# jkxing/EPSM_Mitsuba3

Hardware: AMD Instinct MI355X
Metric: manifold_paths_per_s (higher is better)
Workload: dtype f32

## Files before the change

### epsm_mitsuba3_amd/csrc/epsm_backward_cp.hip

```cpp
#include <stdlib.h>
#include <string.h>

#define EPSM_FAST_RCP64
#include "epsm_fused.h"
#include "epsm_cp_core.h"
#include "epsm_wave_scatter.h"

using namespace epsm;

namespace {

#ifndef EPSM_CP_THREADS
#define EPSM_CP_THREADS 256
#endif
#ifndef EPSM_CP_OCC
#define EPSM_CP_OCC 3
#endif
#ifndef EPSM_CP_ROWS_FLOAT
#define EPSM_CP_ROWS_FLOAT 2064
#endif
#ifndef EPSM_CP_ROWS_FIXED
#define EPSM_CP_ROWS_FIXED 1184
#endif
#ifndef EPSM_CP_QUEUE
#define EPSM_CP_QUEUE 192
#endif
#ifndef EPSM_CP_BLOCKS
#define EPSM_CP_BLOCKS (1 << 20)
#endif
constexpr int kThreads = EPSM_CP_THREADS, kWaves = kThreads / 64, kQueueCap = EPSM_CP_QUEUE;
constexpr int kKeys = 6;
constexpr int kStashFirstItem = 64;
static_assert(kQueueCap - kStashFirstItem >= 128, "the stash needs 128 queue items");

__device__ __forceinline__ int div_small(int lane, int c) {
    const int inv = c == 1 ? 65536 : c == 2 ? 32768 : c == 3 ? 21846 : c == 4 ? 16384 : 13108;
    return (lane * inv) >> 16;
}

__device__ __forceinline__ int up1_bits(int v) { return __builtin_amdgcn_update_dpp(v, v, 0x138, 0xf, 0xf, false); }
__device__ __forceinline__ int down1_bits(int v) { return __builtin_amdgcn_update_dpp(v, v, 0x130, 0xf, 0xf, false); }
__device__ __forceinline__ float up1(float v) { return __int_as_float(up1_bits(__float_as_int(v))); }
__device__ __forceinline__ float down1(float v) { return __int_as_float(down1_bits(__float_as_int(v))); }
__device__ __forceinline__ int up1(int v) { return up1_bits(v); }
__device__ __forceinline__ int down1(int v) { return down1_bits(v); }
__device__ __forceinline__ uint32_t up1(uint32_t v) { return (uint32_t) up1_bits((int) v); }
__device__ __forceinline__ uint32_t down1(uint32_t v) { return (uint32_t) down1_bits((int) v); }
__device__ __forceinline__ V2<float> up1(V2<float> v) { return mk2<float>(up1(v.x), up1(v.y)); }
__device__ __forceinline__ M2<float> up1(M2<float> m) { M2<float> o; o.a = up1(m.a); o.b = up1(m.b); o.c = up1(m.c); o.d = up1(m.d); return o; }
__device__ __forceinline__ V3<float> down1(V3<float> v) { return mk3<float>(down1(v.x), down1(v.y), down1(v.z)); }
__device__ __forceinline__ V3<float> up1(V3<float> v) { return mk3<float>(up1(v.x), up1(v.y), up1(v.z)); }

template <bool PACKED> struct Records {
    const FusedArgs &F;
    const PtrTable &P;
    int64_t i;
    __device__ __forceinline__ cp::Own<float> own(int k) const {
        cp::Own<float> o;
        const VertexPtrs<float> &v = P.v[k - 1];
        const Geo<float> g = load_geo(v, i);
        const Nrm<float> nr = load_nrm(v, i, g.b0, g.b1);
        o.x = g.x; o.e1 = g.e1; o.e2 = g.e2; o.b0 = g.b0; o.b1 = g.b1;
        o.n = nr.n; o.dn1 = nr.dn1; o.dn2 = nr.dn2; o.eta = lds_(v.eta, i); o.light = load3(v.light, i);
        return o;
    }
    __device__ __forceinline__ Geo<float> geo(int k) const { return load_geo(P.v[k - 1], i); }
    __device__ __forceinline__ V3<float> cam() const { return load3(F.g.cam, i); }
    __device__ __forceinline__ uint32_t tri_id(int k) const { return lds_(P.s[k - 1].tri, i); }
    __device__ __forceinline__ void b0b1(int k, float &b0, float &b1) const { b0 = lds_(P.v[k - 1].b0, i); b1 = lds_(P.v[k - 1].b1, i); }
    __device__ __forceinline__ bool emit(int k, uint32_t &etri, float &eb0, float &eb1, float &ew) const {
        const uint32_t *p = P.s[k - 1].emit;
        if (!p) return false;
        const U4 e4 = load_u4(p, i);
        etri = e4.x; eb0 = bits_to_float(e4.y); eb1 = bits_to_float(e4.z); ew = bits_to_float(e4.w);
        return true;
    }
    __device__ __forceinline__ void aux(int k, uint32_t &bid, V3<float> &dhf) const {
        bid = kNoIndex; dhf = zero3<float>();
        if (!F.galpha || !P.s[k - 1].aux) return;
        const U4 a4 = load_u4(P.s[k - 1].aux, i);
        bid = a4.x; dhf = mk3<float>(bits_to_float(a4.y), bits_to_float(a4.z), bits_to_float(a4.w));
    }
    __device__ __forceinline__ uint32_t flag_word() const {
        if (PACKED) return lds_(F.pk_flags, i);
        uint32_t w = 0;
        for (int k = 1; k <= F.K; ++k) {
            const VertexPtrs<float> &v = P.v[k - 1];
            const uint32_t b = lds_(v.bsdf, i);
            w |= (((b & kBsdfDiffuse) ? 1u : 0u) | ((b & kBsdfNull) ? 2u : 0u) | (lds_(v.active, i) ? 4u : 0u) |
                  (lds_(v.active_em, i) ? 8u : 0u) | (lds_(v.ismesh, i) ? 16u : 0u)) << (5 * (k - 1));
        }
        return w;
    }
};

template <typename Table> struct Emitter {
    const FusedArgs &F;
    const Table &T;
    WaveQueue<kQueueCap> &Q;

    template <int ROWS>
    __device__ __forceinline__ void push(bool valid, const uint32_t key[ROWS], const V3<float> val[ROWS]) const {
        Q.template push_rows<ROWS>(T, valid, key, val);
    }
    __device__ __forceinline__ V3<float> fin(V3<float> g) const {
        return mk3<float>(finalize(g.x, F.g.clip), finalize(g.y, F.g.clip), finalize(g.z, F.g.clip));
    }
    __device__ __forceinline__ static bool tri_ok(const U4 &t, int64_t V) {
        return t.x < (uint64_t) V && t.y < (uint64_t) V && t.z < (uint64_t) V;
    }
    __device__ __forceinline__ void rows3(bool v, V3<float> vals[3], uint32_t a, uint32_t b, uint32_t c) const {
        const uint32_t keys[3] = {a, b, c};
        push<3>(v, keys, vals);
    }
    __device__ __forceinline__ void group(bool v, V3<float> g, float w0, float w1, uint32_t a, uint32_t b, uint32_t c) const {
        if (__ballot(v) == 0ull) return;
        V3<float> vals[3] = {g * w0, g * w1, g * (1.f - w0 - w1)};
        rows3(v, vals, a, b, c);
    }
    __device__ __forceinline__ void vertex(bool on, bool live, bool d1, V3<float> Gx, V3<float> gn, V3<float> gm, V3<float> glight,
                                           V3<float> gdiff, V3<float> dp, V3<float> n, V3<float> e1, V3<float> e2, float b0, float b1,
                                           float nb0, float nb1, uint32_t bid, V3<float> dhf, float eb0, float eb1, float ew,
                                           const U4 &t, const U4 &tn, const U4 &er, const U4 &sh, const U4 &ts) const {
        const V3<float> z = zero3<float>();
        const bool idx_ok = tri_ok(t, F.V), pos_ok = idx_ok && (t.w & kModePos);
        gn = fin(gn);
        const bool gn_on = on && idx_ok && nz3(gn);
        const float sgn = (t.w & kModeFlip) ? -1.f : 1.f;
        const V3<float> dpf = d1 ? fin(dp) : z;
        {
            const float b2 = 1.f - b0 - b1;
            V3<float> P[3] = {on ? fin(Gx * b0) : z, on ? fin(Gx * b1) : z, on ? fin(Gx * b2) : z};
            if (gn_on && !(t.w & kModeVertexNormals) && pos_ok) {
                const V3<float> d0 = e2 - e1, d1_ = -e1;
                const V3<float> cr = cross(d0, d1_);
                const float il = rsqrt_(dot(cr, cr));
                const V3<float> ch = cr * il;
                const V3<float> cb = (gn - ch * dot(ch, gn)) * (il * sgn);
                const V3<float> d0b = cross(d1_, cb), d1b = cross(cb, d0);
                P[1] = P[1] + d0b; P[2] = P[2] + d1b; P[0] = P[0] - (d0b + d1b);
            }
            if (d1) { P[0] = P[0] + dpf * b0; P[1] = P[1] + dpf * b1; P[2] = P[2] + dpf * b2; }
            const bool v = pos_ok && (nz3(P[0]) || nz3(P[1]) || nz3(P[2]));
            if (__ballot(v) != 0ull) rows3(v, P, t.x, t.y, t.z);
        }
        {
            V3<float> pg = z;
            if (gn_on && (t.w & kModeVertexNormals) && (t.w & kModeNrm)) {
                const float il = rsqrt_(dot(n, n));
                const V3<float> sh_ = n * il;
                pg = (gn - sh_ * dot(sh_, gn)) * (il * sgn);
            }
            const uint32_t V32 = (uint32_t) F.V;
            group(nz3(pg), pg, b0, b1, V32 + t.x, V32 + t.y, V32 + t.z);
        }
        {
            glight = fin(glight);
            const bool v = on && nz3(glight) && tri_ok(er, F.V) && (er.w & kModePos);
            group(v, glight * ew, eb0, eb1, er.x, er.y, er.z);
        }
        {
            gm = fin(gm);
            bool v = on && nz3(gm) && bid < (uint64_t) F.B;
            if (__ballot(v) != 0ull) {
                V3<float> val[1] = {mk3<float>(v ? dot(gm, dhf) : 0.f, 0.f, 0.f)};
                const uint32_t aid[3] = {2u * (uint32_t) F.V + bid, 0u, 0u};
                push<1>(v, aid, val);
            }
        }
        {
            gdiff = fin(gdiff);
            const bool v = live && nz3(gdiff) && tri_ok(tn, F.V) && (tn.w & kModePos);
            group(v, gdiff, nb0, nb1, tn.x, tn.y, tn.z);
        }
        {
            const float dis = bits_to_float(sh.w);
            const bool v = d1 && nz3(dpf) && tri_ok(ts, F.V) && (ts.w & kModePos) && dis != 0.f;
            group(v, dpf * dis, bits_to_float(sh.y), bits_to_float(sh.z), ts.x, ts.y, ts.z);
        }
    }
};

struct LaneId { int q, c, k; uint32_t plan; int loc; };
struct Rounds {
    int cls[kKeys + 1], rb[kKeys + 1];
    const uint16_t *perm;
    const uint32_t *plan;
    __device__ __forceinline__ LaneId lane_of(int r, int lane) const {
        LaneId L;
        int q = 0;
#pragma unroll
        for (int t = 1; t < kKeys; ++t) if (r >= rb[t]) q = t;
        int cls_q = cls[0], n_q = cls[1] - cls[0], rb_q = rb[0];
#pragma unroll
        for (int t = 1; t < kKeys; ++t) if (q == t) { cls_q = cls[t]; n_q = cls[t + 1] - cls[t]; rb_q = rb[t]; }
        const int c = q > 0 ? q : 1, ppr = 64 / c;
        const int j = div_small(lane, c), k = lane - j * c + 1;
        const int idx = (r - rb_q) * ppr + j;
        const bool lane_on = r >= 0 && r < rb[kKeys] && j < ppr && idx < n_q;
        const int loc = lane_on ? (int) perm[cls_q + idx] : 0;
        L.q = q; L.c = c; L.k = k; L.loc = loc;
        L.plan = lane_on ? plan[loc] : 0u;
        return L;
    }
};

typedef float F2v __attribute__((ext_vector_type(2)));
typedef float F3v __attribute__((ext_vector_type(3)));
struct GeoFetch {
    F4v o0, o1, o2, o3, o4, o5;
    float o_lz;
    F4v p0, p1, p2;
    F4v n0, n1, n2;
    float gx, gy;
};
struct AddrFetch {
    F4v q6;
    F4v q7;
    U4 sh;
};
__device__ __forceinline__ F2v ld2(const float *p) { return *(const __attribute__((address_space(1))) F2v *) p; }
struct WinBase {
    const float *verts, *rays;
    const uint32_t *shadow;
    const uint32_t *list;
    int64_t base;
    uint32_t pix0, rem0;
    float rcp_spp, rcp_res;
    bool small;
};
__device__ __forceinline__ WinBase win_base(const FusedArgs &F, int64_t base) {
    WinBase B;
    B.base = base;
    B.verts = F.pk_verts + base * F.pk_path_stride;
    B.rays = F.pk_rays + base * F.pk_ray_stride;
    B.shadow = F.pk_shadow ? F.pk_shadow + 4 * base : nullptr;
    B.list = F.pk_list ? F.pk_list + base : nullptr;
    const int64_t p0 = F.tin.path_offset + base, q0 = p0 / F.tin.spp;
    B.small = (int64_t) F.tin.res * F.tin.res < (1 << 24) && q0 + 4096 < (1 << 24) && F.tin.spp < (1 << 20);
    B.pix0 = (uint32_t) q0; B.rem0 = (uint32_t) (p0 - q0 * F.tin.spp);
    B.rcp_spp = 1.f / (float) F.tin.spp; B.rcp_res = 1.f / (float) F.tin.res;
    return B;
}
__device__ __forceinline__ void divmod24(uint32_t x, uint32_t d, float rcp_d, uint32_t &qo, uint32_t &ro) {
    uint32_t q = (uint32_t) ((float) x * rcp_d);
    int32_t r = (int32_t) x - (int32_t) (q * d);
    if (r < 0) { --q; r += (int32_t) d; }
    if (r >= (int32_t) d) { ++q; r -= (int32_t) d; }
    qo = q; ro = (uint32_t) r;
}
struct LaneRole { bool ok, first, live, end_next, d1, act1; uint32_t loc; const float *rec, *rays; const uint32_t *shadow; int64_t path; };
template <bool LIST>
__device__ __forceinline__ LaneRole role_of(const FusedArgs &F, const LaneId &L, const WinBase &B) {
    LaneRole R;
    R.ok = L.plan != 0u;
    R.first = L.k == 1;
    R.live = R.ok && L.q > 0;
    R.end_next = R.live && L.k == L.c && L.k + 1 <= cp::plan_nv(L.plan);
    R.d1 = R.ok && R.first && cp::plan_diffuse1(L.plan);
    R.act1 = (L.plan & cp::kPlanActive1) != 0;
    R.loc = (uint32_t) L.loc;
    if (LIST && B.list) {
        const int64_t i = R.ok ? (int64_t) lds_(B.list, (int64_t) R.loc) : 0;
        R.path = i;
        R.rec = F.pk_verts + i * F.pk_path_stride + (L.k - 1) * kRecWords;
        R.rays = F.pk_rays + i * F.pk_ray_stride;
        R.shadow = F.pk_shadow ? F.pk_shadow + 4 * i : nullptr;
        return R;
    }
    R.path = -1;
    R.rec = B.verts + (uint32_t) (R.loc * (uint32_t) F.pk_path_stride + (uint32_t) (L.k - 1) * (uint32_t) kRecWords);
    R.rays = B.rays + (uint32_t) F.pk_ray_stride * R.loc;
    R.shadow = B.shadow ? B.shadow + 4 * R.loc : nullptr;
    return R;
}
__device__ __attribute__((noinline)) int64_t pixel_offset_large(int64_t path, int spp, int res, int img_width) {
    const int64_t pix = path / spp, y = pix / res;
    return y * img_width + (pix - y * res);
}
__device__ __forceinline__ const float *pixel_grad(const TangentIn &A, const WinBase &B, uint32_t loc, int64_t path = -1) {
    if (path >= 0) return A.grad_img + pixel_offset_large(A.path_offset + path, A.spp, A.res, A.img_width) * A.img_channels + 3;
    if (!B.small) return A.grad_img + pixel_offset_large(A.path_offset + B.base + loc, A.spp, A.res, A.img_width) * A.img_channels + 3;
    int64_t y, x;
    {
        uint32_t q1, r1, yy, xx;
        divmod24(B.rem0 + loc, (uint32_t) A.spp, B.rcp_spp, q1, r1);
        divmod24(B.pix0 + q1, (uint32_t) A.res, B.rcp_res, yy, xx);
        y = yy; x = xx;
    }
    return A.grad_img + (y * A.img_width + x) * A.img_channels + 3;
}
typedef __attribute__((address_space(3))) const F4v LdsF4;
typedef __attribute__((address_space(3))) F4v LdsF4w;
template <bool LIST>
__device__ __forceinline__ void geo_issue_rest(GeoFetch &X, const FusedArgs &F, const LaneId &L, const WinBase &B) {
    const LaneRole R = role_of<LIST>(F, L, B);
    if (R.ok && R.first) {
        const float *rays = R.rays;
        X.p0 = ldq(rays, 0); X.p1 = ldq(rays, 1); X.p2 = ldq(rays, 2);
        const F2v g = ld2(pixel_grad(F.tin, B, R.loc, R.path));
        X.gx = g.x; X.gy = g.y;
    }
    if (R.end_next) {
        const float *nx = R.rec + kRecWords;
        X.n0 = ldq(nx, 0); X.n1 = ldq(nx, 1); X.n2 = ldq(nx, 2);
    }
}
template <int VARIANT, bool LIST>
__device__ __forceinline__ void addr_issue(AddrFetch &A, const FusedArgs &F, const LaneId &L, const WinBase &B) {
    const LaneRole R = role_of<LIST>(F, L, B);
    if (R.live) {
        const bool wN = VARIANT == EPSM_VARIANT_MANIFOLD && cp::plan_a(L.plan, L.k);
        if (F.galpha || wN) A.q7 = ldq(R.rec, 7);
        if (wN) A.q6 = ldq(R.rec, 6);
    }
    if (R.d1 && R.shadow) A.sh = load_u4(R.shadow, 0);
}

template <int VARIANT, bool LIST>
__device__ __forceinline__ void own_issue(GeoFetch &X, AddrFetch &A, const FusedArgs &F, const LaneId &L, const WinBase &B) {
    const LaneRole R = role_of<LIST>(F, L, B);
    if (R.live || R.d1) { X.o0 = ldq(R.rec, 0); X.o1 = ldq(R.rec, 1); X.o2 = ldq(R.rec, 2); }
    if (R.live) { X.o3 = ldq(R.rec, 3); X.o4 = ldq(R.rec, 4); X.o5 = ldq(R.rec, 5); }
    addr_issue<VARIANT, LIST>(A, F, L, B);
}
__device__ __forceinline__ void fetch_zero(GeoFetch &X, AddrFetch &A) {
    const F4v z4 = {0.f, 0.f, 0.f, 0.f};
    X.o0 = X.o1 = X.o2 = X.o3 = X.o4 = X.o5 = X.p0 = X.p1 = X.p2 = X.n0 = X.n1 = X.n2 = z4;
    X.o_lz = X.gx = X.gy = 0.f;
    A.q6 = A.q7 = z4; A.sh.x = kNoIndex; A.sh.y = A.sh.z = A.sh.w = 0u;
}

#ifndef EPSM_CP_WINDOW
#define EPSM_CP_WINDOW 2048
#endif

template <int VARIANT, int DMODE, bool PACKED, bool FLOAT_ROWS, int kWindow, bool DROP>
__global__ __launch_bounds__(kThreads, EPSM_CP_OCC) void epsm_backward_cp_kernel(FusedArgs F, int dcols, int64_t windows_per_block, int window) {
    constexpr bool kFloatRows = FLOAT_ROWS;
    constexpr int kRowsFixed = kWindow > 1024 ? EPSM_CP_ROWS_FIXED - 224 * ((kWindow - 1024) / 1024) : EPSM_CP_ROWS_FIXED;
    constexpr int kRowsFloat = kWindow > 1024 ? EPSM_CP_ROWS_FLOAT - 384 * ((kWindow - 1024) / 1024) : EPSM_CP_ROWS_FLOAT;
    typedef LdsTable<kFloatRows ? kRowsFloat : kRowsFixed, typename std::conditional<kFloatRows, AccFloat, AccFixed64>::type> Table;
    constexpr int kTableSize = Table::kTableSize;
    __shared__ uint32_t s_keys[kTableSize];
    __shared__ typename Table::Val s_vals[kTableSize * 3];
    __shared__ int s_used;
    __shared__ QItem s_queue[kWaves][kQueueCap];
    __shared__ PtrTable s_ptrs;
    float *const my_rep = F.rep ? F.rep + (blockIdx.x % (unsigned) F.replicas) * F.rep_stride : nullptr;
    const Table T{s_keys, s_vals, &s_used, my_rep ? my_rep : F.gpos, my_rep ? my_rep + 3 * F.V : F.gnrm,
                  my_rep ? my_rep + 6 * F.V : F.galpha, (uint32_t) F.V};
    const int wv = threadIdx.x >> 6, lane = threadIdx.x & 63;
    WaveQueue<kQueueCap> Q{s_queue[wv], 0};
    const Emitter<Table> E{F, T, Q};
    if (!PACKED && threadIdx.x < F.K) { s_ptrs.v[threadIdx.x] = F.g.v[threadIdx.x]; s_ptrs.s[threadIdx.x] = F.s[threadIdx.x]; }
    constexpr int kPer = (kWindow + kThreads - 1) / kThreads;
    constexpr int kSortKeys = DROP ? kKeys + 1 : kKeys;
    constexpr bool kList = DROP && PACKED;
    constexpr int kStride = kPer * kWaves, kEntries = kSortKeys * kStride;
    __shared__ uint32_t s_plan[kWindow];
    __shared__ uint16_t s_perm[kWindow];
    __shared__ int s_cnt[kEntries];
    __shared__ int s_cls[kKeys + 2];
    V3<float> gd_acc = zero3<float>();
    const int64_t n_slots = (kList && F.pk_list) ? (int64_t) lds_(F.pk_list_count, (int64_t) 0) : F.g.N;
    const int64_t n_windows = (n_slots + window - 1) / window;
    if (kList && !F.rep_done && (int64_t) blockIdx.x * windows_per_block >= n_windows) return;
    T.clear();
#pragma unroll 1
    for (int64_t wi = 0; wi < windows_per_block; ++wi) {
        const int64_t win = (int64_t) blockIdx.x * windows_per_block + wi;
        if (win >= n_windows) break;
        const int64_t base = win * window;
        const WinBase WB = win_base(F, base);
        int key[kPer], rank[kPer];
        {
            uint32_t fw[kPer];
#pragma unroll
            for (int j = 0; j < kPer; ++j) {
                int64_t p = base + j * kThreads + threadIdx.x;
                if (kList && F.pk_list) p = p < n_slots ? (int64_t) lds_(F.pk_list, p) : -1;
                const Records<PACKED> R{F, s_ptrs, (p >= 0 && p < F.g.N) ? p : F.g.N - 1};
                fw[j] = (j * kThreads + (int) threadIdx.x < window && p >= 0 && p < F.g.N) ? R.flag_word() : 0u;
            }
#pragma unroll
            for (int j = 0; j < kPer; ++j) {
                const int loc = j * kThreads + threadIdx.x;
                const int64_t p = base + loc;
                const bool in = loc < window && p < n_slots;
                uint32_t w = fw[j];
                if (F.K < 5) w &= (1u << (5 * F.K)) - 1u;
                uint32_t plan = VARIANT == EPSM_VARIANT_MANIFOLD ? cp::manifold_plan(w) : cp::caustic_plan(w);
                plan = in ? (plan | cp::kPlanInRange | ((w & 4u) ? cp::kPlanActive1 : 0u)) : 0u;
                const bool none = kSortKeys > kKeys && (!in || (cp::plan_m(plan) == 0 && !cp::plan_diffuse1(plan)));
                key[j] = none ? kKeys : cp::plan_m(plan);
                if (loc < window) s_plan[loc] = plan;
            }
        }
#pragma unroll
        for (int j = 0; j < kPer; ++j) {
            const bool has = j * kThreads + (int) threadIdx.x < window;
#pragma unroll
            for (int q = 0; q < kSortKeys; ++q) {
                const unsigned long long m = __ballot(has && key[j] == q);
                if (key[j] == q) rank[j] = __builtin_amdgcn_mbcnt_hi((unsigned) (m >> 32), __builtin_amdgcn_mbcnt_lo((unsigned) m, 0u));
                if (lane == 0) s_cnt[(q * kPer + j) * kWaves + wv] = __popcll(m);
            }
        }
        __syncthreads();
        if (wv == 0) {
            int carry = 0;
#pragma unroll
            for (int q0 = 0; q0 < kEntries; q0 += 64) {
                const int q = q0 + lane;
                const int c = q < kEntries ? s_cnt[q] : 0;
                int inc = c;
#pragma unroll
                for (int off = 1; off < 64; off <<= 1) { const int t = __shfl_up(inc, off); if (lane >= off) inc += t; }
                if (q < kEntries) {
                    s_cnt[q] = carry + inc - c;
                    if (q % kStride == 0) s_cls[q / kStride] = carry + inc - c;
                }
                carry += __shfl(inc, 63);
            }
            if (lane == 0) s_cls[kSortKeys] = window;
        }
        __syncthreads();
#pragma unroll
        for (int j = 0; j < kPer; ++j) {
            const int loc = j * kThreads + threadIdx.x;
            if (loc < window) s_perm[s_cnt[(key[j] * kPer + j) * kWaves + wv] + rank[j]] = (uint16_t) loc;
        }
        __syncthreads();
        Rounds RS;
        RS.perm = s_perm; RS.plan = s_plan;
#pragma unroll
        for (int q = 0; q <= kKeys; ++q) RS.cls[q] = __builtin_amdgcn_readfirstlane(s_cls[q]);
        RS.rb[0] = 0;
#pragma unroll
        for (int q = 0; q < kKeys; ++q) {
            const int c = q > 0 ? q : 1, ppr = 64 / c;
            RS.rb[q + 1] = RS.rb[q] + (RS.cls[q + 1] - RS.cls[q] + ppr - 1) / ppr;
        }
        const int n_rounds = RS.rb[kKeys];
        LaneId L = RS.lane_of(wv, lane);
        GeoFetch Xp; AddrFetch Ap;
        fetch_zero(Xp, Ap);
        if (PACKED) own_issue<VARIANT, kList>(Xp, Ap, F, L, WB);
#pragma unroll 1
        for (int r = wv; r < n_rounds; r += kWaves) {
            const int q = L.q, c = L.c, k = L.k;
            const uint32_t plan = L.plan;
            const bool ok = plan != 0u, first = k == 1;
            const int64_t i = base + L.loc;
            const Records<PACKED> R{F, s_ptrs, i};
            const int nv = cp::plan_nv(plan);
            const bool live = ok && q > 0;
            const bool has_next = live && k + 1 <= nv;
            const bool d1 = ok && first && cp::plan_diffuse1(plan);
            const bool act1 = (plan & cp::kPlanActive1) != 0;

            asm volatile("; EPSM_MARK round_begin");
            cp::Own<float> own;
            own.x = own.e1 = own.e2 = own.n = own.dn1 = own.dn2 = own.light = zero3<float>();
            own.b0 = own.b1 = own.eta = 0.f;
            cp::Nbr<float> prev, next;
            prev.x = prev.e1 = prev.e2 = next.x = next.e1 = next.e2 = zero3<float>();
            V2<float> dk = mk2<float>(0.f, 0.f);
            V3<float> dp = zero3<float>();
            const bool wN = VARIANT == EPSM_VARIANT_MANIFOLD && live && cp::plan_a(plan, k);
            float nb0 = 0.f, nb1 = 0.f;
            uint32_t tid_own = kNoIndex, tid_next = kNoIndex, bid = kNoIndex, etri = kNoIndex;
            V3<float> dhf = zero3<float>();
            float eb0 = 0.f, eb1 = 0.f, ew = 0.f;
            U4 sh; sh.x = kNoIndex; sh.y = sh.z = sh.w = 0u;
            if (PACKED) {
                GeoFetch X;
                {
                    const F4v z4 = {0.f, 0.f, 0.f, 0.f};
                    X.o0 = X.o1 = X.o2 = X.o3 = X.o4 = X.o5 = X.p0 = X.p1 = X.p2 = X.n0 = X.n1 = X.n2 = z4;
                    X.o_lz = X.gx = X.gy = 0.f;
                }
                geo_issue_rest<kList>(X, F, L, WB);
                X.o0 = Xp.o0; X.o1 = Xp.o1; X.o2 = Xp.o2; X.o3 = Xp.o3; X.o4 = Xp.o4; X.o5 = Xp.o5;
                Q.drain_full_groups(T);
                {
                    AddrFetch A0;
                    const F4v z4s = {0.f, 0.f, 0.f, 0.f};
                    A0.q6 = A0.q7 = z4s; A0.sh.x = kNoIndex; A0.sh.y = A0.sh.z = A0.sh.w = 0u;
                    A0 = Ap;
                    float *st = (float *) s_queue[wv] + 4 * kStashFirstItem + 8 * lane;
                    const bool has_sh = d1 && F.pk_shadow;
                    const F4v shv = {__uint_as_float(A0.sh.x), __uint_as_float(A0.sh.y), __uint_as_float(A0.sh.z), __uint_as_float(A0.sh.w)};
                    *(LdsF4w *) st = has_sh ? shv : A0.q6; *(LdsF4w *) (st + 4) = A0.q7;
                    X.o_lz = A0.q7.x;
                }
                if (live) {
                    const Geo<float> g = geo_from(X.o0, X.o1, X.o2);
                    const Nrm<float> nr = nrm_from(X.o3, X.o4, X.o5, g.b0, g.b1);
                    own.x = g.x; own.e1 = g.e1; own.e2 = g.e2; own.b0 = g.b0; own.b1 = g.b1;
                    own.n = nr.n; own.dn1 = nr.dn1; own.dn2 = nr.dn2;
                    own.eta = X.o3.w; own.light = mk3<float>(X.o5.z, X.o5.w, X.o_lz);
                }
                if (d1 && !live) { own.b0 = X.o2.y; own.b1 = X.o2.z; }
                if (live || d1) tid_own = __float_as_uint(X.o2.w);
                if (c > 1) {
                    const V3<float> ux = up1(own.x), ue1 = up1(own.e1), ue2 = up1(own.e2);
                    const V3<float> dx = down1(own.x), de1 = down1(own.e1), de2 = down1(own.e2);
                    if (live && !first) { prev.x = ux; prev.e1 = ue1; prev.e2 = ue2; }
                    if (has_next && k < c) { next.x = dx; next.e1 = de1; next.e2 = de2; }
                }
                if (live && first) prev.x = mk3<float>(X.p0.x, X.p0.y, X.p0.z);
                if (has_next && k == c) {
                    const Geo<float> gq = geo_from(X.n0, X.n1, X.n2);
                    next.x = gq.x; next.e1 = gq.e1; next.e2 = gq.e2;
                    nb0 = gq.b0; nb1 = gq.b1; tid_next = __float_as_uint(X.n2.w);
                }
                if (ok && first) {
                    const V3<float> ro = mk3<float>(X.p0.x, X.p0.y, X.p0.z), rd = mk3<float>(X.p0.w, X.p1.x, X.p1.y),
                                    rdx = mk3<float>(X.p1.z, X.p1.w, X.p2.x), rdy = mk3<float>(X.p2.y, X.p2.z, X.p2.w);
                    V3<float> p0 = zero3<float>(), p1 = p0, p2 = p0;
                    const bool need_tri = act1 && (live || d1);
                    if (need_tri) { p0 = mk3<float>(X.o0.x, X.o0.y, X.o0.z); p1 = mk3<float>(X.o0.w, X.o1.x, X.o1.y); p2 = mk3<float>(X.o1.z, X.o1.w, X.o2.x); }
                    const Tangent t = tangent_from(ro, rd, rdx, rdy, X.gx, X.gy, p0, p1, p2, need_tri);
                    dk = mk2<float>(t.db0, t.db1);
                    dp = t.dp;
                    gd_acc = gd_acc + t.gd;
                }
            } else {
                if (live) {
                    own = R.own(k);
                    if (first) prev.x = R.cam();
                    else { const Geo<float> g = R.geo(k - 1); prev.x = g.x; prev.e1 = g.e1; prev.e2 = g.e2; }
                    tid_own = R.tri_id(k);
                    if (wN) R.emit(k, etri, eb0, eb1, ew);
                    if (F.galpha) R.aux(k, bid, dhf);
                }
                if (has_next) {
                    const Geo<float> g = R.geo(k + 1);
                    next.x = g.x; next.e1 = g.e1; next.e2 = g.e2; nb0 = g.b0; nb1 = g.b1;
                    tid_next = R.tri_id(k + 1);
                }
                if (d1) {
                    R.b0b1(1, own.b0, own.b1);
                    tid_own = R.tri_id(1);
                    if (s_ptrs.s[0].shadow) sh = load_u4(s_ptrs.s[0].shadow, i);
                }
                if (DMODE == kTangentsInKernel) {
                    if (ok && first) {
                        const Tangent t = first_vertex_tangent(F.tin, i, s_ptrs.v[0].p0, s_ptrs.v[0].p1, s_ptrs.v[0].p2, act1);
                        dk = mk2<float>(t.db0, t.db1);
                        dp = t.dp;
                        gd_acc = gd_acc + t.gd;
                    }
                } else {
                    if (ok && (first || DMODE == kTangentsFullRows)) dk = load_d<float, DMODE == kTangentsFullRows>(F.g, i, k, dcols);
                    if (ok && first) dp = load3(F.g.dldp, i);
                }
            }
            cp::Pts<float> pts;
            pts.x = own.x; pts.n = own.n; pts.light = own.light; pts.eta = own.eta; pts.xp = prev.x; pts.xn = next.x;
            const V3<float> keep_e1 = own.e1, keep_e2 = own.e2;
            const float kb0 = own.b0, kb1 = own.b1;

            asm volatile("; EPSM_MARK solve");
            V3<float> Gx = zero3<float>(), gn = Gx, gm = Gx, glight = Gx, gdiff = Gx;
            bool emit_vertex = live;
            AddrFetch A;
            {
                const F4v z4 = {0.f, 0.f, 0.f, 0.f};
                A.q6 = A.q7 = z4;
                A.sh.x = kNoIndex; A.sh.y = A.sh.z = A.sh.w = 0u;
            }
            if (VARIANT == EPSM_VARIANT_MANIFOLD) {
                cp::MSeeds<float> sd;
                sd.sN = sd.sC = mk2<float>(0.f, 0.f); sd.useN = sd.useC = sd.fC = false;
                if (q > 0) {
                    const bool wC = live && cp::plan_b(plan, k);
                    const cp::MBlocks<float> e = cp::manifold_blocks(own, prev, next, wN, has_next);
                    cp::MFwd<float> f = cp::manifold_fwd(e, dk, true, cp::mfwd_zero<float>(), e.Aup, wN, has_next);
#pragma unroll 1
                    for (int s = 2; s <= c; ++s) {
                        cp::MFwd<float> pf;
                        pf.z = up1(f.z); pf.Sinv = up1(f.Sinv); pf.zN = mk2<float>(0.f, 0.f);
                        const M2<float> pAup = up1(e.Aup);
                        const cp::MFwd<float> g = cp::manifold_fwd(e, dk, false, pf, pAup, wN, has_next);
                        if (k == s) f = g;
                    }
                    cp::MBwd<float> mine; mine.q = mk2<float>(0.f, 0.f); mine.W = 0;
#pragma unroll 1
                    for (int s = c; s >= 1; --s) {
                        cp::MBwd<float> nb;
                        nb.q = mk2<float>(down1(mine.q.x), down1(mine.q.y)); nb.W = down1(mine.W);
                        if (s == c) { nb.q = mk2<float>(0.f, 0.f); nb.W = 0; }
                        cp::MBwd<float> m2;
                        const cp::MSeeds<float> s2 = cp::manifold_bwd(e, f, nb, wN, wC, has_next, m2);
                        if (k == s) { sd = s2; mine = m2; }
                    }
                }
                __builtin_amdgcn_sched_barrier(0);
                if (PACKED) {
                    const float *st = (const float *) s_queue[wv] + 4 * kStashFirstItem + 8 * lane;
                    const F4v a = *(LdsF4 *) st;
                    A.q7 = *(LdsF4 *) (st + 4);
                    if (d1 && F.pk_shadow) { A.sh.x = __float_as_uint(a.x); A.sh.y = __float_as_uint(a.y); A.sh.z = __float_as_uint(a.z); A.sh.w = __float_as_uint(a.w); }
                    else A.q6 = a;
                    asm volatile("s_waitcnt lgkmcnt(0)" ::: "memory");
                }
                __builtin_amdgcn_sched_barrier(0);
                if (q > 0) {
                    const cp::MOut<float> o = cp::manifold_contract(pts, sd, has_next);
                    const V3<float> from_next = down1(o.GP);
                    Gx = k < c ? o.Gx - from_next : o.Gx;
                    gn = o.gn; gm = o.gm; glight = o.glight; gdiff = o.gdiff;
                }
            } else {
                cp::CFwd<float> f = cp::cfwd_zero<float>();
                bool poisoned = false;
                const int idstar = cp::plan_idstar(plan);
                if (q > 0) {
                    const cp::CBlocks<float> e = cp::caustic_blocks(own, prev, next, first);
                    f = cp::caustic_fwd(e, dk, true, cp::cfwd_zero<float>(), e.Aup);
#pragma unroll 1
                    for (int s = 2; s <= c; ++s) {
                        cp::CFwd<float> pf = cp::cfwd_zero<float>();
                        pf.v = up1(f.v); pf.r = up1(f.r);
                        const M2<float> pAup = up1(e.Aup);
                        const cp::CFwd<float> g = cp::caustic_fwd(e, dk, false, pf, pAup);
                        if (k == s) f = g;
                    }
                    const unsigned long long bad = __ballot(live && k == idstar && !f.fin);
                    const unsigned long long seg = ((1ull << c) - 1ull) << (lane - (k - 1));
                    poisoned = (bad & seg) != 0ull;
                }
                __builtin_amdgcn_sched_barrier(0);
                if (PACKED) {
                    const float *st = (const float *) s_queue[wv] + 4 * kStashFirstItem + 8 * lane;
                    const F4v a = *(LdsF4 *) st;
                    A.q7 = *(LdsF4 *) (st + 4);
                    if (d1 && F.pk_shadow) { A.sh.x = __float_as_uint(a.x); A.sh.y = __float_as_uint(a.y); A.sh.z = __float_as_uint(a.z); A.sh.w = __float_as_uint(a.w); }
                    else A.q6 = a;
                    asm volatile("s_waitcnt lgkmcnt(0)" ::: "memory");
                }
                __builtin_amdgcn_sched_barrier(0);
                if (q > 0) {
                    const cp::COut<float> o = cp::caustic_finish(pts, f, first, live && k <= idstar, live && k == idstar, live && cp::plan_b(plan, k));
                    const V3<float> from_next = down1(o.gxp_prev);
                    Gx = k < c ? o.Gx + from_next : o.Gx;
                    gn = o.gn; gm = o.gm; gdiff = o.gdiff;
                    emit_vertex = live && k <= idstar && !poisoned;
                }
            }
            asm volatile("; EPSM_MARK addressing");
            float fb0 = kb0, fb1 = kb1;
            if (PACKED) {
                if (live) {
                    if (F.galpha) dhf = mk3<float>(A.q7.y, A.q7.z, A.q7.w);
                    if (wN) { etri = __float_as_uint(A.q6.x); eb0 = A.q6.y; eb1 = A.q6.z; ew = A.q6.w; }
                }
                if (d1 && F.pk_shadow) sh = A.sh;
                if (c > 1) {
                    const float db0 = down1(kb0), db1 = down1(kb1);
                    const uint32_t dt = down1(tid_own);
                    if (has_next && k < c) { nb0 = db0; nb1 = db1; tid_next = dt; }
                }
            }
            const U4 t_own = table_row(F.tab, tid_own), t_next = table_row(F.tab, tid_next);
            const U4 er = table_row(F.tab, etri), t_sh = table_row(F.tab, sh.x);
            asm volatile("; EPSM_MARK prefetch");
            const LaneId Ln = RS.lane_of(r + kWaves, lane);
            if (PACKED) { fetch_zero(Xp, Ap); own_issue<VARIANT, kList>(Xp, Ap, F, Ln, WB); }
            asm volatile("; EPSM_MARK emit");
            if (PACKED) bid = (t_own.w >> 8) - 1u;
            E.vertex(emit_vertex && q > 0, live, d1, Gx, gn, gm, glight, gdiff, dp, pts.n, keep_e1, keep_e2, fb0, fb1,
                     nb0, nb1, bid, dhf, eb0, eb1, ew, t_own, t_next, er, sh, t_sh);
            asm volatile("; EPSM_MARK round_end");
            L = Ln;
        }
        Q.drain(T);
        if (wi + 1 < windows_per_block && win + 1 < n_windows) T.flush();
    }
    T.flush(true);
    if (DMODE == kTangentsInKernel && F.grad_o_sum) {
        __shared__ float s_part[kWaves][3];
        float sx = -gd_acc.x, sy = -gd_acc.y, sz = -gd_acc.z;
#pragma unroll
        for (int off = 32; off > 0; off >>= 1) { sx += __shfl_down(sx, off, 64); sy += __shfl_down(sy, off, 64); sz += __shfl_down(sz, off, 64); }
        if (lane == 0) { s_part[wv][0] = sx; s_part[wv][1] = sy; s_part[wv][2] = sz; }
        __syncthreads();
        if (threadIdx.x < 3) {
            float tot = 0.f;
            for (int w = 0; w < kWaves; ++w) tot += s_part[w][threadIdx.x];
            atomicAdd((my_rep ? my_rep + 6 * F.V + F.B : F.grad_o_sum) + threadIdx.x, tot);
        }
    }
    if (my_rep && F.rep_done) {
        __shared__ int s_last;
        const unsigned rix = blockIdx.x % (unsigned) F.replicas;
        __threadfence();
        __syncthreads();
        if (threadIdx.x == 0) {
            const unsigned members = ((unsigned) F.rep_blocks - rix + (unsigned) F.replicas - 1u) / (unsigned) F.replicas;
            s_last = atomicAdd(F.rep_done + rix, 1u) + 1u == members;
        }
        __syncthreads();
        if (s_last) {
            __threadfence();
            const int64_t n = 6 * F.V + F.B + 3;
            constexpr int kU = 8;
            for (int64_t e0 = threadIdx.x; e0 < n; e0 += (int64_t) kThreads * kU) {
                float v[kU];
#pragma unroll
                for (int u = 0; u < kU; ++u) {
                    const int64_t e = e0 + (int64_t) u * kThreads;
                    v[u] = e < n ? __hip_atomic_load(my_rep + e, __ATOMIC_RELAXED, __HIP_MEMORY_SCOPE_AGENT) : 0.f;
                }
#pragma unroll
                for (int u = 0; u < kU; ++u) {
                    const int64_t e = e0 + (int64_t) u * kThreads;
                    if (e < n && v[u] != 0.f) {
                        float *dst = e < 3 * F.V ? F.gpos + e : e < 6 * F.V ? F.gnrm + (e - 3 * F.V) : e < 6 * F.V + F.B ? (F.galpha ? F.galpha + (e - 6 * F.V) : nullptr)
                                                                                                         : (F.grad_o_sum ? F.grad_o_sum + (e - 6 * F.V - F.B) : nullptr);
                        if (dst && adds_something(v[u])) atomicAdd(dst, v[u]);
                        my_rep[e] = 0.f;
                    }
                }
            }
            if (threadIdx.x == 0) F.rep_done[rix] = 0u;
        }
    }
}

template <int VARIANT, int DMODE, bool PACKED>
hipError_t launch(const FusedArgs &F0, int dcols, hipStream_t s) {
    FusedArgs F = F0;
    const bool small = F.g.N <= fused_option(EPSM_OPT_SMALL_WAVEFRONT_PATHS);
#ifndef EPSM_CP_SLOTS
#define EPSM_CP_SLOTS 768
#endif
#ifndef EPSM_CP_WINDOW_CAUSTIC
#define EPSM_CP_WINDOW_CAUSTIC 2048
#endif
    constexpr int kSmall = 1024, kSlots = EPSM_CP_SLOTS;
    constexpr int kLargeRT = VARIANT == EPSM_VARIANT_MANIFOLD ? EPSM_CP_WINDOW : EPSM_CP_WINDOW_CAUSTIC;
    constexpr int kLarge = kLargeRT > 1024 ? EPSM_CP_WINDOW : 1024;
    int window = kLargeRT;
    if (small) {
        const int64_t w = ((F.g.N + kSlots - 1) / kSlots + 63) / 64 * 64;
        window = (int) (w < 128 ? 128 : w > kSmall ? kSmall : w);
    }
    const int64_t windows = (F.g.N + window - 1) / window;
    const int64_t blocks = windows < EPSM_CP_BLOCKS ? windows : EPSM_CP_BLOCKS;
    const int64_t per = (windows + blocks - 1) / blocks;
    F.rep = nullptr; F.replicas = 1; F.rep_stride = 0; F.rep_done = nullptr; F.rep_blocks = 0;
    if (small) {
        const int64_t stride = (6 * F.V + F.B + 3 + 63) / 64 * 64;
        int64_t R = blocks / 16;
        if (R > 32) R = 32;
        if (R * stride * 4 > (int64_t) kReplicaBudget) R = (int64_t) kReplicaBudget / (stride * 4);
        if (R >= 4 && fused_option(EPSM_OPT_REPLICAS) != 0) {
            const hipError_t e = fused_workspace(s, (size_t) (R * stride * 4), &F.rep);
            if (e != hipSuccess) return e;
            if (F.rep) {
                F.replicas = (int) R; F.rep_stride = stride;
                F.rep_blocks = (int) blocks;
                F.rep_done = fused_option(EPSM_OPT_ONE_LAUNCH) != 0 ? (uint32_t *) ((char *) F.rep + kReplicaBudget) : nullptr;
            }
        }
    }
    const bool float_rows = !(F.g.clip <= 1.f);
    const bool drop = DMODE != kTangentsInKernel || F.grad_o_sum == nullptr;
#define EPSM_CP_LAUNCH(FLOAT_ROWS_, WINDOW_, DROP_) \
    hipLaunchKernelGGL((epsm_backward_cp_kernel<VARIANT, DMODE, PACKED, FLOAT_ROWS_, WINDOW_, (DROP_) || DMODE != kTangentsInKernel>), \
                       dim3((unsigned) blocks), dim3(kThreads), 0, s, F, dcols, per, window)
    if (float_rows) {
        if (small) { if (drop) EPSM_CP_LAUNCH(true, kSmall, true); else EPSM_CP_LAUNCH(true, kSmall, false); }
        else { if (drop) EPSM_CP_LAUNCH(true, kLarge, true); else EPSM_CP_LAUNCH(true, kLarge, false); }
    } else {
        if (small) { if (drop) EPSM_CP_LAUNCH(false, kSmall, true); else EPSM_CP_LAUNCH(false, kSmall, false); }
        else { if (drop) EPSM_CP_LAUNCH(false, kLarge, true); else EPSM_CP_LAUNCH(false, kLarge, false); }
    }
#undef EPSM_CP_LAUNCH
    hipError_t le = hipGetLastError();
    if (le == hipSuccess && F.rep && !F.rep_done) {
        const int64_t n = 6 * F.V + F.B + 3;
        hipLaunchKernelGGL(reduce_replicas_kernel, dim3((unsigned) ((n + 255) / 256)), dim3(256), 0, s, F.rep, F.replicas, F.rep_stride,
                           F.V, F.B, F.gpos, F.gnrm, F.galpha, F.grad_o_sum);
        le = hipGetLastError();
    }
    if (le != hipSuccess && F.rep) fused_workspace_invalidate(s);
    return le;
}
template <int VARIANT, bool PACKED> hipError_t launch_d(int dmode, const FusedArgs &F, int dcols, hipStream_t s) {
    switch (dmode) {
        case kTangentsTwoColumns: return launch<VARIANT, kTangentsTwoColumns, PACKED>(F, dcols, s);
        case kTangentsFullRows: return launch<VARIANT, kTangentsFullRows, PACKED>(F, dcols, s);
        default: return launch<VARIANT, kTangentsInKernel, PACKED>(F, dcols, s);
    }
}

}

namespace epsm {

hipError_t launch_backward_cp(int variant, int dmode, bool packed, const FusedArgs &F, int dcols, hipStream_t s) {
    if (packed) {
        return variant == EPSM_VARIANT_MANIFOLD ? launch<EPSM_VARIANT_MANIFOLD, kTangentsInKernel, true>(F, dcols, s)
                                                : launch<EPSM_VARIANT_MANIFOLD_CAUSTIC, kTangentsInKernel, true>(F, dcols, s);
    }
    return variant == EPSM_VARIANT_MANIFOLD ? launch_d<EPSM_VARIANT_MANIFOLD, false>(dmode, F, dcols, s)
                                            : launch_d<EPSM_VARIANT_MANIFOLD_CAUSTIC, false>(dmode, F, dcols, s);
}

}
```

Measured before the change: 9.416 billion.

## Make geometry loads unconditional using a per-window dummy record

Predicated global loads of ray, neighbour and own-record data are replaced by unconditional loads. Inactive lanes point at a valid per-window substitute record (the first listed path or the window base), so no lane reads out of bounds. The change also drops the zero-initialisation of fetch structs and Own fields, always computes the own geometry, hoists ppr into the class-select loop, and makes the wave index scalar via readfirstlane. The aim is to remove divergent branches and exec-mask handling around loads and to cut register setup work. In exchange it issues more memory traffic from inactive lanes, and non-live lanes now receive values derived from real data instead of zeros, which downstream code must ignore.

Result: faster. 9.697 billion, median of 6 (+3.0%).

```diff
diff --git a/epsm_mitsuba3_amd/csrc/epsm_backward_cp.hip b/epsm_mitsuba3_amd/csrc/epsm_backward_cp.hip
--- a/epsm_mitsuba3_amd/csrc/epsm_backward_cp.hip
+++ b/epsm_mitsuba3_amd/csrc/epsm_backward_cp.hip
@@ -191,10 +191,10 @@
         int q = 0;
 #pragma unroll
         for (int t = 1; t < kKeys; ++t) if (r >= rb[t]) q = t;
-        int cls_q = cls[0], n_q = cls[1] - cls[0], rb_q = rb[0];
-#pragma unroll
-        for (int t = 1; t < kKeys; ++t) if (q == t) { cls_q = cls[t]; n_q = cls[t + 1] - cls[t]; rb_q = rb[t]; }
-        const int c = q > 0 ? q : 1, ppr = 64 / c;
+        int cls_q = cls[0], n_q = cls[1] - cls[0], rb_q = rb[0], ppr = 64;
+#pragma unroll
+        for (int t = 1; t < kKeys; ++t) if (q == t) { cls_q = cls[t]; n_q = cls[t + 1] - cls[t]; rb_q = rb[t]; ppr = 64 / t; }
+        const int c = q > 0 ? q : 1;
         const int j = div_small(lane, c), k = lane - j * c + 1;
         const int idx = (r - rb_q) * ppr + j;
         const bool lane_on = r >= 0 && r < rb[kKeys] && j < ppr && idx < n_q;
@@ -222,6 +222,8 @@
 __device__ __forceinline__ F2v ld2(const float *p) { return *(const __attribute__((address_space(1))) F2v *) p; }
 struct WinBase {
     const float *verts, *rays;
+    const float *sub_rec;
+    int64_t sub_path;
     const uint32_t *shadow;
     const uint32_t *list;
     int64_t base;
@@ -229,10 +231,17 @@
     float rcp_spp, rcp_res;
     bool small;
 };
+template <bool LIST>
 __device__ __forceinline__ WinBase win_base(const FusedArgs &F, int64_t base) {
     WinBase B;
     B.base = base;
     B.verts = F.pk_verts + base * F.pk_path_stride;
+    B.sub_rec = B.verts; B.sub_path = 0;
+    if (LIST && F.pk_list) {
+        const int64_t p = (int64_t) lds_(F.pk_list, base);
+        B.sub_path = (p >= 0 && p < F.g.N) ? p : 0;
+        B.sub_rec = F.pk_verts + B.sub_path * F.pk_path_stride;
+    }
     B.rays = F.pk_rays + base * F.pk_ray_stride;
     B.shadow = F.pk_shadow ? F.pk_shadow + 4 * base : nullptr;
     B.list = F.pk_list ? F.pk_list + base : nullptr;
@@ -259,9 +268,9 @@
     R.end_next = R.live && L.k == L.c && L.k + 1 <= cp::plan_nv(L.plan);
     R.d1 = R.ok && R.first && cp::plan_diffuse1(L.plan);
     R.act1 = (L.plan & cp::kPlanActive1) != 0;
-    R.loc = (uint32_t) L.loc;
+    R.loc = R.ok ? (uint32_t) L.loc : 0u;
     if (LIST && B.list) {
-        const int64_t i = R.ok ? (int64_t) lds_(B.list, (int64_t) R.loc) : 0;
+        const int64_t i = R.ok ? (int64_t) lds_(B.list, (int64_t) R.loc) : B.sub_path;
         R.path = i;
         R.rec = F.pk_verts + i * F.pk_path_stride + (L.k - 1) * kRecWords;
         R.rays = F.pk_rays + i * F.pk_ray_stride;
@@ -295,16 +304,12 @@
 template <bool LIST>
 __device__ __forceinline__ void geo_issue_rest(GeoFetch &X, const FusedArgs &F, const LaneId &L, const WinBase &B) {
     const LaneRole R = role_of<LIST>(F, L, B);
-    if (R.ok && R.first) {
-        const float *rays = R.rays;
-        X.p0 = ldq(rays, 0); X.p1 = ldq(rays, 1); X.p2 = ldq(rays, 2);
-        const F2v g = ld2(pixel_grad(F.tin, B, R.loc, R.path));
-        X.gx = g.x; X.gy = g.y;
-    }
-    if (R.end_next) {
-        const float *nx = R.rec + kRecWords;
-        X.n0 = ldq(nx, 0); X.n1 = ldq(nx, 1); X.n2 = ldq(nx, 2);
-    }
+    const float *rays = R.rays;
+    X.p0 = ldq(rays, 0); X.p1 = ldq(rays, 1); X.p2 = ldq(rays, 2);
+    const F2v g = ld2(pixel_grad(F.tin, B, R.loc, R.path));
+    X.gx = g.x; X.gy = g.y;
+    const float *nx = R.end_next ? R.rec + kRecWords : B.sub_rec;
+    X.n0 = ldq(nx, 0); X.n1 = ldq(nx, 1); X.n2 = ldq(nx, 2);
 }
 template <int VARIANT, bool LIST>
 __device__ __forceinline__ void addr_issue(AddrFetch &A, const FusedArgs &F, const LaneId &L, const WinBase &B) {
@@ -320,14 +325,13 @@
 template <int VARIANT, bool LIST>
 __device__ __forceinline__ void own_issue(GeoFetch &X, AddrFetch &A, const FusedArgs &F, const LaneId &L, const WinBase &B) {
     const LaneRole R = role_of<LIST>(F, L, B);
-    if (R.live || R.d1) { X.o0 = ldq(R.rec, 0); X.o1 = ldq(R.rec, 1); X.o2 = ldq(R.rec, 2); }
-    if (R.live) { X.o3 = ldq(R.rec, 3); X.o4 = ldq(R.rec, 4); X.o5 = ldq(R.rec, 5); }
+    const float *rec012 = (R.live || R.d1) ? R.rec : B.sub_rec, *rec345 = R.live ? R.rec : B.sub_rec;
+    X.o0 = ldq(rec012, 0); X.o1 = ldq(rec012, 1); X.o2 = ldq(rec012, 2);
+    X.o3 = ldq(rec345, 3); X.o4 = ldq(rec345, 4); X.o5 = ldq(rec345, 5);
     addr_issue<VARIANT, LIST>(A, F, L, B);
 }
 __device__ __forceinline__ void fetch_zero(GeoFetch &X, AddrFetch &A) {
     const F4v z4 = {0.f, 0.f, 0.f, 0.f};
-    X.o0 = X.o1 = X.o2 = X.o3 = X.o4 = X.o5 = X.p0 = X.p1 = X.p2 = X.n0 = X.n1 = X.n2 = z4;
-    X.o_lz = X.gx = X.gy = 0.f;
     A.q6 = A.q7 = z4; A.sh.x = kNoIndex; A.sh.y = A.sh.z = A.sh.w = 0u;
 }
 
@@ -350,7 +354,7 @@
     float *const my_rep = F.rep ? F.rep + (blockIdx.x % (unsigned) F.replicas) * F.rep_stride : nullptr;
     const Table T{s_keys, s_vals, &s_used, my_rep ? my_rep : F.gpos, my_rep ? my_rep + 3 * F.V : F.gnrm,
                   my_rep ? my_rep + 6 * F.V : F.galpha, (uint32_t) F.V};
-    const int wv = threadIdx.x >> 6, lane = threadIdx.x & 63;
+    const int wv = __builtin_amdgcn_readfirstlane((int) (threadIdx.x >> 6)), lane = threadIdx.x & 63;
     WaveQueue<kQueueCap> Q{s_queue[wv], 0};
     const Emitter<Table> E{F, T, Q};
     if (!PACKED && threadIdx.x < F.K) { s_ptrs.v[threadIdx.x] = F.g.v[threadIdx.x]; s_ptrs.s[threadIdx.x] = F.s[threadIdx.x]; }
@@ -372,7 +376,7 @@
         const int64_t win = (int64_t) blockIdx.x * windows_per_block + wi;
         if (win >= n_windows) break;
         const int64_t base = win * window;
-        const WinBase WB = win_base(F, base);
+        const WinBase WB = win_base<kList>(F, base);
         int key[kPer], rank[kPer];
         {
             uint32_t fw[kPer];
@@ -462,8 +466,10 @@
 
             asm volatile("; EPSM_MARK round_begin");
             cp::Own<float> own;
-            own.x = own.e1 = own.e2 = own.n = own.dn1 = own.dn2 = own.light = zero3<float>();
-            own.b0 = own.b1 = own.eta = 0.f;
+            if (!PACKED) {
+                own.x = own.e1 = own.e2 = own.n = own.dn1 = own.dn2 = own.light = zero3<float>();
+                own.b0 = own.b1 = own.eta = 0.f;
+            }
             cp::Nbr<float> prev, next;
             prev.x = prev.e1 = prev.e2 = next.x = next.e1 = next.e2 = zero3<float>();
             V2<float> dk = mk2<float>(0.f, 0.f);
@@ -476,11 +482,6 @@
             U4 sh; sh.x = kNoIndex; sh.y = sh.z = sh.w = 0u;
             if (PACKED) {
                 GeoFetch X;
-                {
-                    const F4v z4 = {0.f, 0.f, 0.f, 0.f};
-                    X.o0 = X.o1 = X.o2 = X.o3 = X.o4 = X.o5 = X.p0 = X.p1 = X.p2 = X.n0 = X.n1 = X.n2 = z4;
-                    X.o_lz = X.gx = X.gy = 0.f;
-                }
                 geo_issue_rest<kList>(X, F, L, WB);
                 X.o0 = Xp.o0; X.o1 = Xp.o1; X.o2 = Xp.o2; X.o3 = Xp.o3; X.o4 = Xp.o4; X.o5 = Xp.o5;
                 Q.drain_full_groups(T);
@@ -495,14 +496,13 @@
                     *(LdsF4w *) st = has_sh ? shv : A0.q6; *(LdsF4w *) (st + 4) = A0.q7;
                     X.o_lz = A0.q7.x;
                 }
-                if (live) {
+                {
                     const Geo<float> g = geo_from(X.o0, X.o1, X.o2);
                     const Nrm<float> nr = nrm_from(X.o3, X.o4, X.o5, g.b0, g.b1);
                     own.x = g.x; own.e1 = g.e1; own.e2 = g.e2; own.b0 = g.b0; own.b1 = g.b1;
                     own.n = nr.n; own.dn1 = nr.dn1; own.dn2 = nr.dn2;
                     own.eta = X.o3.w; own.light = mk3<float>(X.o5.z, X.o5.w, X.o_lz);
                 }
-                if (d1 && !live) { own.b0 = X.o2.y; own.b1 = X.o2.z; }
                 if (live || d1) tid_own = __float_as_uint(X.o2.w);
                 if (c > 1) {
                     const V3<float> ux = up1(own.x), ue1 = up1(own.e1), ue2 = up1(own.e2);
```
